# Renmusxd/IsingMonteCarlo

Measured on AMD Instinct MI355X. Metric: spin-op updates/sec (whole node), 32×32 TFIM, 1024 replicas at 1/2/4/8 GPUs, higher is better.
Workload: dtype u32 op words, f64 acceptance arithmetic

## Files before the change

isingmontecarlo_amd/csrc/sse_cluster.hip.h:

```cpp
#pragma once

namespace sse {

#define SSE_CLW 16
#define SSE_CL_MAX_VARS 4095u
#define SSE_CLE_TWO (1u << 28)
#define SSE_CLE_LONG (1u << 29)
#define SSE_CLE_CUT (1u << 31)
#define SSE_CL_TOUCHED (1u << 24)

typedef __attribute__((address_space(3))) uint32_t sse_lds_u32;
typedef __attribute__((address_space(3))) uint16_t sse_lds_u16;
typedef __attribute__((address_space(3))) uint8_t sse_lds_u8;
#define LDS32B(a) (*(sse_lds_u32 *)(uintptr_t)(a))
#define LDS16B(a) (*(sse_lds_u16 *)(uintptr_t)(a))
#define LDS8B(a) (*(sse_lds_u8 *)(uintptr_t)(a))
__device__ __forceinline__ void lds_cas32(uint32_t addr, uint32_t expect, uint32_t val) {
    (void)__hip_atomic_compare_exchange_strong((sse_lds_u32 *)(uintptr_t)addr, &expect, val, __ATOMIC_RELAXED, __ATOMIC_RELAXED, __HIP_MEMORY_SCOPE_WORKGROUP);
}

struct ClLds {
    uint32_t o_tab;
    uint32_t o_state;
    uint32_t o_touch;
    uint32_t o_misc;
    uint32_t o_chn;
    uint32_t o_chtr;
    uint32_t o_ent;
    uint32_t o_frozen, o_froot;
    uint32_t o_parent;
    uint32_t end;
    __host__ __device__ __forceinline__ void carve(uint32_t N, uint32_t nwords, uint32_t Nb, uint32_t ufcap, bool has_long) {
        uint32_t base = 0;
        o_tab = base; base += Nb + 1u;
        o_state = base; base += nwords;
        o_touch = base; base += nwords;
        o_misc = base; base += 16u;
        o_chn = base; base += SSE_MAX_CHUNKS;
        o_chtr = base; base += SSE_MAX_CHUNKS;
        o_ent = base; base += (uint32_t)SSE_CLW * (N + 1u);
        o_frozen = base; base += has_long ? (ufcap + 31u) / 32u : 0u;
        o_froot = base; base += has_long ? (ufcap + 31u) / 32u : 0u;
        o_parent = base;
        end = base + (ufcap + 1u) / 2u;
    }
};
static inline __host__ __device__ bool cl_ids_fit(uint32_t N, uint32_t S, uint32_t ufcap) {
    return S < ufcap && S < 65535u && ((size_t)S + 31) / 32 <= (size_t)SSE_CLW * (N + 1);
}
static inline __host__ __device__ uint32_t cl_list_cap(uint32_t N, uint32_t S) {
    const size_t tab = (size_t)SSE_CLW * (N + 1), bits = ((size_t)S + 31) / 32;
    return bits < tab ? (uint32_t)(2 * (tab - bits)) : 0u;
}

__device__ __forceinline__ uint32_t cl_entry(const DevBatch &B, uint32_t b, uint32_t ce) {
    if (b < B.E) return (ce & SSE_CE_VAR_MASK) | (((ce >> 15) & SSE_CE_VAR_MASK) << 13) | SSE_CLE_TWO;
    const uint32_t s1 = b - B.E;
    if (s1 < B.N) return s1 | (s1 << 13) | SSE_CLE_CUT;
    const uint32_t v = s1 - B.N;
    return v | (v << 13) | SSE_CLE_LONG;
}

__device__ __forceinline__ uint32_t cl_union_wave(const UFA<false> &uf, uint32_t a, uint32_t b) {
    for (;;) {
        uint32_t xa = a, xb = b, pa = uf.get(a), pb = uf.get(b);
        while ((pa != xa) | (pb != xb)) { xa = pa; xb = pb; pa = uf.get(xa); pb = uf.get(xb); }
        if (a != xa) uf.set(a, xa);
        if (b != xb) uf.set(b, xb);
        if (xa == xb) return xa;
        const uint32_t lo = min(xa, xb), hi = max(xa, xb);
        uf.set(hi, lo);
        SSE_WAVE_FENCE();
        if (uf.get(hi) == lo) return lo;
        a = xa; b = xb;
    }
}

#ifndef SSE_CL_FIND_LEVELS
#define SSE_CL_FIND_LEVELS 4
#endif
template <int K, bool HAS_LONG, int PHASE>
__global__ __launch_bounds__(SSE_CLW * 64, 4) void cluster_kernel(DevBatch B, SweepArgs A) {
    constexpr int W = SSE_CLW, NT = W * 64;
    constexpr uint32_t TS = 64u * K;
    static_assert(K == 2 || K == 4, "ids are stored two rows per dword");
    ClLds L;
    L.carve(B.N, B.nwords, B.Nb, B.lds_ufcap, HAS_LONG);
    const int tid = threadIdx.x, lane = tid & 63, wave = __builtin_amdgcn_readfirstlane(tid >> 6);
    const uint32_t r = blockIdx.x;
    const uint32_t N = B.N, nwords = B.nwords;
    const int n = (int)B.n[r];
    const uint32_t C = B.ntrans[r], M = B.cutoff[r], err = B.err[r];
    if (err) return;
    const uint32_t S = N + C + (uint32_t)(W - 1) * N;
    if (n == 0 || C == 0u || !cl_ids_fit(N, S, B.lds_ufcap)) {
        if (tid == 0) B.aux[r] = 1u;
        return;
    }
    UFA<false> uf;
    uf.gparent = nullptr; uf.gfrozen = nullptr; uf.gfroot = nullptr;
    uf.o_parent = L.o_parent; uf.o_frozen = L.o_frozen; uf.o_froot = L.o_froot;
    uint64_t epoch = B.epoch[r];
    uint32_t *ops = B.ops + (size_t)r * B.stride;
    uint32_t *ids = B.segs + (size_t)r * B.stride;
    const bool DEFER = A.defer_flips != 0u && B.flipb != nullptr;
    uint4 *msk = reinterpret_cast<uint4 *>(ids + B.stride / 2u);

    SSE_STAMP_INIT;
    for (uint32_t i = tid; i < nwords; i += NT) { LDSW(L.o_state, i) = B.state[(size_t)r * nwords + i]; LDSW(L.o_touch, i) = 0u; }
    for (uint32_t i = tid; i <= B.Nb; i += NT)
        LDSW(L.o_tab, i) = i == 0u ? (N | (N << 13)) : cl_entry(B, i - 1u, i - 1u < B.E ? B.edges_compact[i - 1u] : 0u);
    for (uint32_t i = tid; i < 2 * SSE_MAX_CHUNKS; i += NT) LDSW(L.o_chn, i) = B.chunks[(size_t)r * 2 * SSE_MAX_CHUNKS + i];
    if (tid == 0) { LDSW(L.o_misc, MISC_NCLUST) = 0u; LDSW(L.o_misc, MISC_ANYFROZEN) = 0u; LDSW(L.o_misc, MISC_LOOP_A) = 0u; }
    for (uint32_t i = tid; i < (uint32_t)W * (N + 1u); i += NT) {
        const uint32_t w2 = i / (N + 1u), v = i - w2 * (N + 1u);
        LDSW(L.o_ent, i) = v == N ? S : (w2 == 0u ? v : N + C + (w2 - 1u) * N + v);
    }
    for (uint32_t i = tid; i < S / 2u + 1u; i += NT) LDSW(L.o_parent, i) = (2u * i) | ((2u * i + 1u) << 16);
    if constexpr (HAS_LONG) for (uint32_t i = tid; i < (S + 31u) / 32u; i += NT) uf.bits_clear(i);
    __syncthreads();

    const uint32_t used = (M + B.CH - 1u) / B.CH;
    const uint32_t q = (used + W - 1u) / W;
    const uint32_t c0 = min((uint32_t)wave * q, used), c1 = min(c0 + q, used);
    uint32_t cutbase = 0;
    for (uint32_t c = lane; c < c0; c += 64) cutbase += LDSW(L.o_chtr, c);
    for (int off = 32; off > 0; off >>= 1) cutbase += __shfl_xor(cutbase, off);
    cutbase = (uint32_t)__builtin_amdgcn_readfirstlane((int)cutbase);
    const uint32_t pbeg = c0 * B.CH, pend = min(c1 * B.CH, M);
    const uint32_t lds0 = (uint32_t)(uintptr_t)(sse_lds_u32 *)lds_raw;
    const uint32_t ent_b = lds0 + 4u * (L.o_ent + (uint32_t)wave * (N + 1u));
    const uint32_t par_b = lds0 + 4u * L.o_parent;

    SSE_STAMP(0);
    {
        uint32_t cutnext = N + cutbase;
        uint32_t wnext[K], idpend[K / 2];
        uint4 mpend[K];
#pragma unroll
        for (int j = 0; j < K; ++j) { wnext[j] = row_ld(ops, pbeg + (uint32_t)(j * 64 + lane)); mpend[j] = make_uint4(0u, 0u, 0u, 0u); }
#pragma unroll
        for (int j = 0; j < K / 2; ++j) idpend[j] = 0u;
        uint32_t pprev = pbeg;
        for (uint32_t p0 = pbeg; p0 < pend; p0 += TS) {
            uint32_t e[K];
            {
                uint32_t word[K];
#pragma unroll
                for (int j = 0; j < K; ++j) word[j] = wnext[j];
#pragma unroll
                for (int j = 0; j < K; j += 2) if (!SSE_DBG(B, 1u)) row_st(ids, (pprev >> 1) + (uint32_t)(j * 32 + lane), idpend[j / 2]);
                if (DEFER) { if (lane == 0) {
#pragma unroll
                    for (int j = 0; j < K; ++j) msk[(pprev >> 6) + (uint32_t)j] = mpend[j];
                } }
                pprev = p0;
                const uint32_t pn0 = p0 + TS < pend ? p0 + TS : p0;
#pragma unroll
                for (int j = 0; j < K; ++j) wnext[j] = row_ld(ops, pn0 + (uint32_t)(j * 64 + lane));
#pragma unroll
                for (int j = 0; j < K; ++j) e[j] = LDS32B(lds0 + 4u * (word[j] >> 4));
            }
            uint32_t ua[K], uc[K], adra[K], adrc[K];
#pragma unroll
            for (int j = 0; j < K; ++j) {
                const uint32_t aa = ent_b + 4u * (e[j] & 0x1FFFu), ac = ent_b + 4u * ((e[j] >> 13) & 0x1FFFu);
                adra[j] = aa; adrc[j] = ac;
                const bool iscut = (int32_t)e[j] < 0;
                const uint64_t cutm = sse_ballot(iscut);
                const uint32_t kown = __builtin_amdgcn_mbcnt_hi((uint32_t)(cutm >> 32), __builtin_amdgcn_mbcnt_lo((uint32_t)cutm, 0u));
                if (iscut) LDS8B(aa + 2u) = (uint8_t)(kown + 1u);
                SSE_WAVE_FENCE();
                const uint32_t ea = LDS32B(aa), ec = LDS32B(ac);
                LDS8B(aa + 3u) = (uint8_t)1; LDS8B(ac + 3u) = (uint8_t)1;
                const uint32_t qa = (ea >> 16) & 0xFFu, qc = (ec >> 16) & 0xFFu;
                uint32_t seg_a = ea & 0xFFFFu, seg_c = ec & 0xFFFFu;
                const uint64_t dup = cutm & sse_ballot(qa != kown + 1u);
                if (!dup) {
                    seg_a = ((qa - 1u) < kown) ? cutnext + (qa - 1u) : seg_a;
                    seg_c = ((qc - 1u) < kown) ? cutnext + (qc - 1u) : seg_c;
                    SSE_WAVE_FENCE();
                    if (iscut) LDS32B(aa) = (cutnext + kown) | SSE_CL_TOUCHED;
                } else {
                    const uint32_t va = e[j] & 0x1FFFu, vc = (e[j] >> 13) & 0x1FFFu;
                    bool lastcut = iscut;
                    uint64_t m = cutm;
                    uint32_t idL = cutnext;
                    while (m) {
                        const int Ls = __ffsll((long long)m) - 1;
                        m &= m - 1;
                        const uint32_t vL = __builtin_amdgcn_readlane(va, Ls);
                        const bool later = lane > Ls, same_a = va == vL;
                        seg_a = (later & same_a) ? idL : seg_a;
                        seg_c = (later & (vc == vL)) ? idL : seg_c;
                        lastcut = lastcut & !((lane < Ls) & same_a);
                        idL++;
                    }
                    SSE_WAVE_FENCE();
                    if (iscut) LDS8B(aa + 2u) = (uint8_t)0;
                    if (iscut & lastcut) LDS16B(aa) = (uint16_t)(cutnext + kown);
                    SSE_WAVE_FENCE();
                }
                if constexpr (HAS_LONG)
                    if (e[j] & SSE_CLE_LONG) uf.frozen_or(seg_a >> 5, 1u << (seg_a & 31));
                cutnext += (uint32_t)popc64(cutm);
                if (DEFER) {
                    mpend[j].x = (uint32_t)cutm; mpend[j].y = (uint32_t)(cutm >> 32);
                    if constexpr (HAS_LONG) { const uint64_t twom = sse_ballot((e[j] & SSE_CLE_TWO) != 0u); mpend[j].z = (uint32_t)twom; mpend[j].w = (uint32_t)(twom >> 32); }
                }
                ua[j] = seg_a; uc[j] = seg_c;
            }
#pragma unroll
            for (int j = 0; j < K; j += 2) idpend[j / 2] = ua[j] | (ua[j + 1] << 16);
#pragma unroll
            for (int j = 0; j < K; ++j) {
                const bool need = ua[j] != uc[j];
                if (!sse_any(need) || SSE_DBG(B, 2u)) continue;
                if (need) {
                    const uint32_t pa = LDS16B(par_b + 2u * ua[j]), pc = LDS16B(par_b + 2u * uc[j]);
                    uint32_t ga = LDS16B(par_b + 2u * pa), gc = LDS16B(par_b + 2u * pc);
                    uint32_t ta = LDS16B(par_b + 2u * ga), tc = LDS16B(par_b + 2u * gc);
#pragma unroll
                    for (int lv = 3; lv < SSE_CL_FIND_LEVELS; ++lv) {
                        const uint32_t na = LDS16B(par_b + 2u * ta), nc = LDS16B(par_b + 2u * tc);
                        ga = ta; gc = tc; ta = na; tc = nc;
                    }
                    const bool found = (ta == ga) & (tc == gc);
                    const bool differ = ga != gc;
                    const bool link = found & differ;
                    uint32_t lo = min(ga, gc);
                    const uint32_t hi = max(ga, gc);
                    if (found & (pa != ga)) { LDS16B(par_b + 2u * ua[j]) = (uint16_t)ga; }
                    if (found & (pc != gc)) { LDS16B(par_b + 2u * uc[j]) = (uint16_t)gc; }
                    if (link) LDS16B(par_b + 2u * hi) = (uint16_t)lo;
                    SSE_WAVE_FENCE();
                    const uint32_t chk = LDS16B(par_b + 2u * hi);
#ifdef SSE_CL_UNION_COUNTERS
                    if (wave == 3) {
                        const uint64_t nf = sse_ballot(!found), cf = sse_ballot(found & link & (chk != lo)), nd = sse_ballot(true);
                        if (lane == (int)(__ffsll((long long)nd) - 1)) {
                            B.dbg[(size_t)r * 16 + 8] += 1; B.dbg[(size_t)r * 16 + 12] += (uint64_t)popc64(nd);
                            if (nf) B.dbg[(size_t)r * 16 + 9] += 1;
                            if (!nf && cf) B.dbg[(size_t)r * 16 + 10] += 1;
                            B.dbg[(size_t)r * 16 + 13] += (uint64_t)popc64(nf); B.dbg[(size_t)r * 16 + 14] += (uint64_t)popc64(cf);
                        }
                    }
#endif
                    if ((!found | (link & (chk != lo))) && !SSE_DBG(B, 16u)) lo = cl_union_wave(uf, pa, pc);
                    lds_cas32(adra[j], ua[j] | SSE_CL_TOUCHED, lo | SSE_CL_TOUCHED);
                    lds_cas32(adrc[j], uc[j] | SSE_CL_TOUCHED, lo | SSE_CL_TOUCHED);
                }
            }
        }
        if (pbeg < pend) {
#pragma unroll
            for (int j = 0; j < K; j += 2) row_st(ids, (pprev >> 1) + (uint32_t)(j * 32 + lane), idpend[j / 2]);
            if (DEFER) { if (lane == 0) {
#pragma unroll
                for (int j = 0; j < K; ++j) msk[(pprev >> 6) + (uint32_t)j] = mpend[j];
            } }
        }
    }
    __syncthreads();
    SSE_STAMP(1);

    for (uint32_t v = tid; v < N; v += NT) {
        uint32_t t = 0;
#pragma unroll 4
        for (uint32_t w2 = 0; w2 < (uint32_t)W; ++w2) {
            const uint32_t x = LDSW(L.o_ent, w2 * (N + 1u) + v);
            t |= x;
            const uint32_t seg_end = x & 0xFFFFu;
            const uint32_t nxt = (w2 + 1u == (uint32_t)W) ? v : N + C + w2 * N + v;
            if (seg_end != nxt) uf_union(uf, seg_end, nxt);
        }
        if (t >> 24) atomicOr(&LDSW(L.o_touch, v >> 5), 1u << (v & 31));
    }
    __syncthreads();
    SSE_STAMP(2);
    for (uint32_t i = tid; i < S; i += NT) {
        const uint32_t root = uf_find_ro(uf, i);
        uf.set(i, root);
        if constexpr (HAS_LONG)
            if ((uf.frozen_get(i >> 5) >> (i & 31)) & 1u) { uf.froot_or(root >> 5, 1u << (root & 31)); LDSW(L.o_misc, MISC_ANYFROZEN) = 1u; }
    }
    const uint32_t o_bits = L.o_ent, o_list = L.o_ent + (S + 31u) / 32u;
    const uint32_t list_cap = cl_list_cap(N, S);
    for (uint32_t i = tid; i < (S + 31u) / 32u; i += NT) LDSW(o_bits, i) = 0u;
    __syncthreads();
    SSE_STAMP(3);
    const Rng rng = make_rng(B, r, epoch);
    uint32_t myclusters = 0;
    for (uint32_t i0 = 0; i0 < S; i0 += NT) {
        const uint32_t i = i0 + tid;
        const bool inr = i < S;
        const uint32_t root = inr ? uf.get(i) : 0xFFFFFFFFu;
        const bool isroot = inr & (root == i);
        if (isroot & (i < N + C)) {
            const bool touched = (i >= N) || ((LDSW(L.o_touch, i >> 5) >> (i & 31)) & 1u);
            if (touched) myclusters++;
        }
        const uint64_t m = sse_ballot(isroot);
        if (m) {
            uint32_t base = 0;
            if (lane == 0) base = atomicAdd(&LDSW(L.o_misc, MISC_LOOP_A), (uint32_t)popc64(m));
            base = (uint32_t)__builtin_amdgcn_readfirstlane((int)base);
            const uint32_t pos = base + popc64(m & lanemask_lt(lane));
            if (isroot && pos < list_cap) LDSH(o_list, pos) = (uint16_t)i;
        }
    }
    __syncthreads();
    const uint32_t nroots = LDSW(L.o_misc, MISC_LOOP_A);
    if (nroots <= list_cap) {
        for (uint32_t k = tid; k < nroots; k += NT) {
            const uint32_t root = LDSH(o_list, k);
            const uint4 o = rng.draw(SSE_TAG_CLUSTER, root);
            const uint32_t isfrozen = HAS_LONG ? (uf.froot_get(root >> 5) >> (root & 31)) & 1u : 0u;
            if (!isfrozen && u01(o.x) < A.prob) atomicOr(&LDSW(o_bits, root >> 5), 1u << (root & 31));
        }
        __syncthreads();
        for (uint32_t i = tid; i < S; i += NT) {
            const uint32_t root = uf.get(i);
            uf.set(i, (LDSW(o_bits, root >> 5) >> (root & 31)) & 1u);
        }
    } else {
        for (uint32_t i = tid; i < S; i += NT) {
            const uint32_t root = uf.get(i);
            const uint4 o = rng.draw(SSE_TAG_CLUSTER, root);
            const uint32_t isfrozen = HAS_LONG ? (uf.froot_get(root >> 5) >> (root & 31)) & 1u : 0u;
            uf.set(i, (!isfrozen && u01(o.x) < A.prob) ? 1u : 0u);
        }
    }
    if (tid == 0) uf.set(S, 0u);
    {
        uint32_t c = myclusters;
        for (int off = 32; off > 0; off >>= 1) c += __shfl_down(c, off);
        if (lane == 0 && c) atomicAdd(&LDSW(L.o_misc, MISC_NCLUST), c);
    }
    __syncthreads();
    SSE_STAMP(4);

    if (DEFER) {
        uint32_t cutnext = N + cutbase;
        uint8_t *fb = B.flipb + (size_t)r * B.stride;
        constexpr int D = 3;
        const uint32_t *mskw = reinterpret_cast<const uint32_t *>(msk);
        uint32_t qid[D][K / 2], qmk[D], bpend[K];
        auto issue = [&](int slot, uint32_t pt) {
            const uint32_t pc = pt < pend ? pt : pbeg;
#pragma unroll
            for (int j = 0; j < K; j += 2) qid[slot][j / 2] = row_ld(ids, (pc >> 1) + (uint32_t)(j * 32 + lane));
            qmk[slot] = row_ld(mskw, (pc >> 6) * 4u + (uint32_t)(lane & 15));
        };
#pragma unroll
        for (int d = 0; d < D; ++d) issue(d, pbeg + (uint32_t)d * TS);
#pragma unroll
        for (int j = 0; j < K; ++j) bpend[j] = 0u;
        uint32_t pprev = pbeg;
        bool first = true;
        for (uint32_t p0 = pbeg; p0 < pend; p0 += TS) {
            uint32_t id2[K / 2];
#pragma unroll
            for (int j = 0; j < K / 2; ++j) id2[j] = qid[0][j];
            const uint32_t mkv = qmk[0];
#pragma unroll
            for (int d = 0; d + 1 < D; ++d) {
#pragma unroll
                for (int j = 0; j < K / 2; ++j) qid[d][j] = qid[d + 1][j];
                qmk[d] = qmk[d + 1];
            }
            if (!first) {
#pragma unroll
                for (int j = 0; j < K; ++j) fb[pprev + (uint32_t)(j * 64 + lane)] = (uint8_t)bpend[j];
            }
            first = false;
            pprev = p0;
            issue(D - 1, p0 + (uint32_t)D * TS);
#pragma unroll
            for (int j = 0; j < K; ++j) {
                const uint64_t cutm = (uint64_t)(uint32_t)__builtin_amdgcn_readlane((int)mkv, 4 * j) | ((uint64_t)(uint32_t)__builtin_amdgcn_readlane((int)mkv, 4 * j + 1) << 32);
                const uint32_t own = __builtin_amdgcn_mbcnt_hi((uint32_t)(cutm >> 32), __builtin_amdgcn_mbcnt_lo((uint32_t)cutm, cutnext));
                const uint32_t idin = (j & 1) ? (id2[j / 2] >> 16) : (id2[j / 2] & 0xFFFFu);
                const uint32_t f1 = LDS16B(par_b + 2u * idin), f2 = LDS16B(par_b + 2u * own);
                uint32_t m_other = (0u - f1) & 0xFu;
                if constexpr (HAS_LONG) {
                    const uint64_t twom = (uint64_t)(uint32_t)__builtin_amdgcn_readlane((int)mkv, 4 * j + 2) | ((uint64_t)(uint32_t)__builtin_amdgcn_readlane((int)mkv, 4 * j + 3) << 32);
                    m_other &= sel64(twom, vgpr_copy_u32(0xFu), vgpr_copy_u32(0x5u));
                }
                bpend[j] = sel64(cutm, f1 | (f2 << 2), m_other);
                cutnext += (uint32_t)popc64(cutm);
            }
        }
        if (pbeg < pend) {
#pragma unroll
            for (int j = 0; j < K; ++j) fb[pprev + (uint32_t)(j * 64 + lane)] = (uint8_t)bpend[j];
        }
    } else
    {
        uint32_t cutnext = N + cutbase;
        const uint32_t E1 = B.E + 1u;
        uint32_t wnext[K], inext[K / 2], wpend[K];
#pragma unroll
        for (int j = 0; j < K; ++j) { wnext[j] = row_ld(ops, pbeg + (uint32_t)(j * 64 + lane)); wpend[j] = wnext[j]; }
#pragma unroll
        for (int j = 0; j < K; j += 2) inext[j / 2] = row_ld(ids, (pbeg >> 1) + (uint32_t)(j * 32 + lane));
        uint32_t pprev = pbeg;
        for (uint32_t p0 = pbeg; p0 < pend; p0 += TS) {
            uint32_t word[K], id2[K / 2];
#pragma unroll
            for (int j = 0; j < K; ++j) word[j] = wnext[j];
#pragma unroll
            for (int j = 0; j < K / 2; ++j) id2[j] = inext[j];
            {
#pragma unroll
                for (int j = 0; j < K; ++j) row_st(ops, pprev + (uint32_t)(j * 64 + lane), wpend[j]);
                pprev = p0;
                const uint32_t pn0 = p0 + TS < pend ? p0 + TS : p0;
#pragma unroll
                for (int j = 0; j < K; ++j) wnext[j] = row_ld(ops, pn0 + (uint32_t)(j * 64 + lane));
#pragma unroll
                for (int j = 0; j < K; j += 2) inext[j / 2] = row_ld(ids, (pn0 >> 1) + (uint32_t)(j * 32 + lane));
            }
            uint32_t f1[K], f2[K];
            uint64_t cutm[K];
#pragma unroll
            for (int j = 0; j < K; ++j) {
                cutm[j] = sse_ballot(((word[j] >> 4) - E1) < N);
                const uint32_t own = __builtin_amdgcn_mbcnt_hi((uint32_t)(cutm[j] >> 32), __builtin_amdgcn_mbcnt_lo((uint32_t)cutm[j], cutnext));
                const uint32_t idin = (j & 1) ? (id2[j / 2] >> 16) : (id2[j / 2] & 0xFFFFu);
                f1[j] = LDS16B(par_b + 2u * idin);
                f2[j] = LDS16B(par_b + 2u * own);
                cutnext += (uint32_t)popc64(cutm[j]);
            }
#pragma unroll
            for (int j = 0; j < K; ++j) {
                const uint32_t allbits = (((word[j] >> 4) - 1u) < B.E) ? 0xFu : 0x5u;
                const uint32_t m_other = (0u - f1[j]) & allbits;
                const uint32_t m_cut = f1[j] | (f2[j] << 2);
                wpend[j] = word[j] ^ sel64(cutm[j], m_cut, m_other);
            }
        }
        if (pbeg < pend) {
#pragma unroll
            for (int j = 0; j < K; ++j) row_st(ops, pprev + (uint32_t)(j * 64 + lane), wpend[j]);
        }
    }
    for (uint32_t i = tid; i < nwords; i += NT) {
        uint32_t x = 0;
        const uint32_t t = LDSW(L.o_touch, i);
        for (uint32_t j = 0; j < 32 && i * 32 + j < N; ++j) x |= (uf.get(i * 32 + j) & 1u) << j;
        LDSW(L.o_state, i) ^= (x & t);
    }
    __syncthreads();
    SSE_STAMP(5);
    const uint32_t nclusters = LDSW(L.o_misc, MISC_NCLUST);
    epoch++;
    uint64_t a0 = 0, a1 = 0, a2 = 0, a3 = 0, a6 = 0;
    if (A.domask & SSE_DO_FREE) {
        const Rng rngf = make_rng(B, r, epoch);
        for (uint32_t i = tid; i < nwords; i += NT) {
            const uint32_t t = LDSW(L.o_touch, i);
            uint32_t s = LDSW(L.o_state, i);
            for (uint32_t j = 0; j < 32 && i * 32 + j < N; ++j)
                if (!((t >> j) & 1u)) {
                    const uint4 o = rngf.draw(SSE_TAG_FREE, i * 32 + j);
                    s = (s & ~(1u << j)) | ((o.x >> 31) << j);
                }
            LDSW(L.o_state, i) = s;
        }
        __syncthreads();
        epoch++;
    }
    if (A.sampling_freq && (A.step0 + 1) % A.sampling_freq == 0) {
        if (tid == 0) LDSW(L.o_misc, MISC_LOOP_A) = 0u;
        __syncthreads();
        uint32_t up = 0;
        for (uint32_t i = tid; i < nwords; i += NT) up += __popc(LDSW(L.o_state, i));
        for (int off = 32; off > 0; off >>= 1) up += __shfl_down(up, off);
        if (lane == 0 && up) atomicAdd(&LDSW(L.o_misc, MISC_LOOP_A), up);
        __syncthreads();
        const long long mag = 2ll * (long long)LDSW(L.o_misc, MISC_LOOP_A) - (long long)N;
        a0 = (uint64_t)n; a1 = 1; a2 = (uint64_t)(mag < 0 ? -mag : mag); a3 = (uint64_t)(mag * mag); a6 = (uint64_t)C;
    }
    for (uint32_t i = tid; i < nwords; i += NT) B.state[(size_t)r * nwords + i] = LDSW(L.o_state, i);
    if (tid == 0) {
        B.epoch[r] = epoch;
        if (DEFER) B.pend[r] = 1u;
        if (A.out_u32) A.out_u32[r] = nclusters;
        uint64_t *acc = B.acc + (size_t)B.acc_row[r] * 8;
        acc[0] += a0; acc[1] += a1; acc[2] += a2; acc[3] += a3; acc[4] += (uint64_t)n; acc[6] += a6;
    }
}

}
```

Measured before the change: 169.4 billion.

## Branchless LDS stores via dummy slot, per-lane spin ops, simpler table setup

```diff
diff --git a/isingmontecarlo_amd/csrc/sse_cluster.hip.h b/isingmontecarlo_amd/csrc/sse_cluster.hip.h
--- a/isingmontecarlo_amd/csrc/sse_cluster.hip.h
+++ b/isingmontecarlo_amd/csrc/sse_cluster.hip.h
@@ -18,6 +18,13 @@
 __device__ __forceinline__ void lds_cas32(uint32_t addr, uint32_t expect, uint32_t val) {
     (void)__hip_atomic_compare_exchange_strong((sse_lds_u32 *)(uintptr_t)addr, &expect, val, __ATOMIC_RELAXED, __ATOMIC_RELAXED, __HIP_MEMORY_SCOPE_WORKGROUP);
 }
+
+__device__ __forceinline__ uint32_t lds_ld16(uint32_t addr) {
+    uint32_t v = LDS16B(addr);
+    asm("" : "+v"(v));
+    return v;
+}
+#define SSE_CL_MISC_DUMMY 12u
 
 struct ClLds {
     uint32_t o_tab;
@@ -53,14 +60,6 @@
     return bits < tab ? (uint32_t)(2 * (tab - bits)) : 0u;
 }
 
-__device__ __forceinline__ uint32_t cl_entry(const DevBatch &B, uint32_t b, uint32_t ce) {
-    if (b < B.E) return (ce & SSE_CE_VAR_MASK) | (((ce >> 15) & SSE_CE_VAR_MASK) << 13) | SSE_CLE_TWO;
-    const uint32_t s1 = b - B.E;
-    if (s1 < B.N) return s1 | (s1 << 13) | SSE_CLE_CUT;
-    const uint32_t v = s1 - B.N;
-    return v | (v << 13) | SSE_CLE_LONG;
-}
-
 __device__ __forceinline__ uint32_t cl_union_wave(const UFA<false> &uf, uint32_t a, uint32_t b) {
     for (;;) {
         uint32_t xa = a, xb = b, pa = uf.get(a), pb = uf.get(b);
@@ -108,13 +107,22 @@
 
     SSE_STAMP_INIT;
     for (uint32_t i = tid; i < nwords; i += NT) { LDSW(L.o_state, i) = B.state[(size_t)r * nwords + i]; LDSW(L.o_touch, i) = 0u; }
-    for (uint32_t i = tid; i <= B.Nb; i += NT)
-        LDSW(L.o_tab, i) = i == 0u ? (N | (N << 13)) : cl_entry(B, i - 1u, i - 1u < B.E ? B.edges_compact[i - 1u] : 0u);
+    if (tid == 0) LDSW(L.o_tab, 0u) = N | (N << 13);
+    for (uint32_t i = tid; i < B.E; i += NT) {
+        const uint32_t ce = B.edges_compact[i];
+        LDSW(L.o_tab, 1u + i) = (ce & SSE_CE_VAR_MASK) | (((ce >> 15) & SSE_CE_VAR_MASK) << 13) | SSE_CLE_TWO;
+    }
+    for (uint32_t v = tid; v < N; v += NT) {
+        const uint32_t vv = v | (v << 13);
+        LDSW(L.o_tab, 1u + B.E + v) = vv | SSE_CLE_CUT;
+        if (1u + B.E + N + v <= B.Nb) LDSW(L.o_tab, 1u + B.E + N + v) = vv | SSE_CLE_LONG;
+    }
     for (uint32_t i = tid; i < 2 * SSE_MAX_CHUNKS; i += NT) LDSW(L.o_chn, i) = B.chunks[(size_t)r * 2 * SSE_MAX_CHUNKS + i];
     if (tid == 0) { LDSW(L.o_misc, MISC_NCLUST) = 0u; LDSW(L.o_misc, MISC_ANYFROZEN) = 0u; LDSW(L.o_misc, MISC_LOOP_A) = 0u; }
-    for (uint32_t i = tid; i < (uint32_t)W * (N + 1u); i += NT) {
-        const uint32_t w2 = i / (N + 1u), v = i - w2 * (N + 1u);
-        LDSW(L.o_ent, i) = v == N ? S : (w2 == 0u ? v : N + C + (w2 - 1u) * N + v);
+    {
+        const uint32_t tb = L.o_ent + (uint32_t)wave * (N + 1u), id0 = wave == 0 ? 0u : N + C + (uint32_t)(wave - 1) * N;
+        for (uint32_t v = (uint32_t)lane; v < N; v += 64u) LDSW(tb, v) = id0 + v;
+        if (lane == 0) LDSW(tb, N) = S;
     }
     for (uint32_t i = tid; i < S / 2u + 1u; i += NT) LDSW(L.o_parent, i) = (2u * i) | ((2u * i + 1u) << 16);
     if constexpr (HAS_LONG) for (uint32_t i = tid; i < (S + 31u) / 32u; i += NT) uf.bits_clear(i);
@@ -131,6 +139,7 @@
     const uint32_t lds0 = (uint32_t)(uintptr_t)(sse_lds_u32 *)lds_raw;
     const uint32_t ent_b = lds0 + 4u * (L.o_ent + (uint32_t)wave * (N + 1u));
     const uint32_t par_b = lds0 + 4u * L.o_parent;
+    const uint32_t dummy_b = vgpr_copy_u32(lds0 + 4u * (L.o_misc + SSE_CL_MISC_DUMMY));
 
     SSE_STAMP(0);
     {
@@ -169,7 +178,8 @@
                 const bool iscut = (int32_t)e[j] < 0;
                 const uint64_t cutm = sse_ballot(iscut);
                 const uint32_t kown = __builtin_amdgcn_mbcnt_hi((uint32_t)(cutm >> 32), __builtin_amdgcn_mbcnt_lo((uint32_t)cutm, 0u));
-                if (iscut) LDS8B(aa + 2u) = (uint8_t)(kown + 1u);
+                const uint32_t acut = iscut ? aa : dummy_b;
+                LDS8B(acut + 2u) = (uint8_t)(kown + 1u);
                 SSE_WAVE_FENCE();
                 const uint32_t ea = LDS32B(aa), ec = LDS32B(ac);
                 LDS8B(aa + 3u) = (uint8_t)1; LDS8B(ac + 3u) = (uint8_t)1;
@@ -180,7 +190,7 @@
                     seg_a = ((qa - 1u) < kown) ? cutnext + (qa - 1u) : seg_a;
                     seg_c = ((qc - 1u) < kown) ? cutnext + (qc - 1u) : seg_c;
                     SSE_WAVE_FENCE();
-                    if (iscut) LDS32B(aa) = (cutnext + kown) | SSE_CL_TOUCHED;
+                    LDS32B(acut) = (cutnext + kown) | SSE_CL_TOUCHED;
                 } else {
                     const uint32_t va = e[j] & 0x1FFFu, vc = (e[j] >> 13) & 0x1FFFu;
                     bool lastcut = iscut;
@@ -197,7 +207,7 @@
                         idL++;
                     }
                     SSE_WAVE_FENCE();
-                    if (iscut) LDS8B(aa + 2u) = (uint8_t)0;
+                    LDS8B(acut + 2u) = (uint8_t)0;
                     if (iscut & lastcut) LDS16B(aa) = (uint16_t)(cutnext + kown);
                     SSE_WAVE_FENCE();
                 }
@@ -217,12 +227,13 @@
                 const bool need = ua[j] != uc[j];
                 if (!sse_any(need) || SSE_DBG(B, 2u)) continue;
                 if (need) {
-                    const uint32_t pa = LDS16B(par_b + 2u * ua[j]), pc = LDS16B(par_b + 2u * uc[j]);
-                    uint32_t ga = LDS16B(par_b + 2u * pa), gc = LDS16B(par_b + 2u * pc);
-                    uint32_t ta = LDS16B(par_b + 2u * ga), tc = LDS16B(par_b + 2u * gc);
+                    const uint32_t xa = par_b + 2u * ua[j], xc = par_b + 2u * uc[j];
+                    const uint32_t pa = lds_ld16(xa), pc = lds_ld16(xc);
+                    uint32_t ga = lds_ld16(par_b + 2u * pa), gc = lds_ld16(par_b + 2u * pc);
+                    uint32_t ta = lds_ld16(par_b + 2u * ga), tc = lds_ld16(par_b + 2u * gc);
 #pragma unroll
                     for (int lv = 3; lv < SSE_CL_FIND_LEVELS; ++lv) {
-                        const uint32_t na = LDS16B(par_b + 2u * ta), nc = LDS16B(par_b + 2u * tc);
+                        const uint32_t na = lds_ld16(par_b + 2u * ta), nc = lds_ld16(par_b + 2u * tc);
                         ga = ta; gc = tc; ta = na; tc = nc;
                     }
                     const bool found = (ta == ga) & (tc == gc);
@@ -230,11 +241,12 @@
                     const bool link = found & differ;
                     uint32_t lo = min(ga, gc);
                     const uint32_t hi = max(ga, gc);
-                    if (found & (pa != ga)) { LDS16B(par_b + 2u * ua[j]) = (uint16_t)ga; }
-                    if (found & (pc != gc)) { LDS16B(par_b + 2u * uc[j]) = (uint16_t)gc; }
-                    if (link) LDS16B(par_b + 2u * hi) = (uint16_t)lo;
+                    const uint32_t xh = par_b + 2u * hi;
+                    LDS16B((found & (pa != ga)) ? xa : dummy_b) = (uint16_t)ga;
+                    LDS16B((found & (pc != gc)) ? xc : dummy_b) = (uint16_t)gc;
+                    LDS16B(link ? xh : dummy_b) = (uint16_t)lo;
                     SSE_WAVE_FENCE();
-                    const uint32_t chk = LDS16B(par_b + 2u * hi);
+                    const uint32_t chk = lds_ld16(xh);
 #ifdef SSE_CL_UNION_COUNTERS
                     if (wave == 3) {
                         const uint64_t nf = sse_ballot(!found), cf = sse_ballot(found & link & (chk != lo)), nd = sse_ballot(true);
@@ -445,11 +457,11 @@
             for (int j = 0; j < K; ++j) row_st(ops, pprev + (uint32_t)(j * 64 + lane), wpend[j]);
         }
     }
-    for (uint32_t i = tid; i < nwords; i += NT) {
-        uint32_t x = 0;
-        const uint32_t t = LDSW(L.o_touch, i);
-        for (uint32_t j = 0; j < 32 && i * 32 + j < N; ++j) x |= (uf.get(i * 32 + j) & 1u) << j;
-        LDSW(L.o_state, i) ^= (x & t);
+    for (uint32_t v0 = (uint32_t)wave * 64u; v0 < N; v0 += NT) {
+        const uint32_t v = v0 + (uint32_t)lane;
+        const uint64_t fm = sse_ballot(v < N && (uf.get(v) & 1u) != 0u);
+        const uint32_t i = (v0 >> 5) + (uint32_t)lane;
+        if (lane < 2 && i < nwords) LDSW(L.o_state, i) ^= (lane ? (uint32_t)(fm >> 32) : (uint32_t)fm) & LDSW(L.o_touch, i);
     }
     __syncthreads();
     SSE_STAMP(5);
@@ -458,15 +470,17 @@
     uint64_t a0 = 0, a1 = 0, a2 = 0, a3 = 0, a6 = 0;
     if (A.domask & SSE_DO_FREE) {
         const Rng rngf = make_rng(B, r, epoch);
-        for (uint32_t i = tid; i < nwords; i += NT) {
-            const uint32_t t = LDSW(L.o_touch, i);
-            uint32_t s = LDSW(L.o_state, i);
-            for (uint32_t j = 0; j < 32 && i * 32 + j < N; ++j)
-                if (!((t >> j) & 1u)) {
-                    const uint4 o = rngf.draw(SSE_TAG_FREE, i * 32 + j);
-                    s = (s & ~(1u << j)) | ((o.x >> 31) << j);
-                }
-            LDSW(L.o_state, i) = s;
+        for (uint32_t v0 = (uint32_t)wave * 64u; v0 < N; v0 += NT) {
+            const uint32_t v = v0 + (uint32_t)lane;
+            const bool isfree = v < N && !((LDSW(L.o_touch, v >> 5) >> (v & 31u)) & 1u);
+            uint32_t bit = 0u;
+            if (isfree) bit = rngf.draw(SSE_TAG_FREE, v).x >> 31;
+            const uint64_t fm = sse_ballot(isfree), bm = sse_ballot(bit != 0u);
+            const uint32_t i = (v0 >> 5) + (uint32_t)lane;
+            if (fm != 0ull && lane < 2 && i < nwords) {
+                const uint32_t f = lane ? (uint32_t)(fm >> 32) : (uint32_t)fm, b = lane ? (uint32_t)(bm >> 32) : (uint32_t)bm;
+                LDSW(L.o_state, i) = (LDSW(L.o_state, i) & ~f) | b;
+            }
         }
         __syncthreads();
         epoch++;
```

After: 172.7 billion, median of 6. 2.0% higher.
